# ubuntuslave/vo_single_camera_sos

Measured on AMD Instinct MI355X. Metric: frame-pairs/sec (detect+match+triangulate+RANSAC) on 640x480 omni, 2000 kpts, higher is better.
Workload: dtype u8/f32/f64

## Files before the change

vo_single_camera_sos_amd/csrc/ransac.hip:

```cpp
#include <type_traits>
#include "common.h"
#include "ransac_core.h"
#include "epnp_core.h"
#include "gp3p_core.h"

namespace {

constexpr int kMaxCam = 8;
constexpr int kHypDoubles = 16;
constexpr int kThreads = 256;
constexpr int kScoreHypChunkMax = 128;

__device__ const double kEye9[9] = {1, 0, 0, 0, 1, 0, 0, 0, 1};
__device__ const double kZero3[3] = {0, 0, 0};

__device__ __forceinline__ uint64_t problem_seed(uint64_t seed, int b) { return seed + (uint64_t)b; }
__device__ __forceinline__ uint64_t problem_seed(const uint64_t* seeds, int b) { return seeds[b]; }

__global__ __launch_bounds__(kThreads) void ransac_prepare_kernel(const int32_t* __restrict__ cam,
                                                                  const int32_t* __restrict__ n_arr, int stride,
                                                                  int ncam, int32_t* __restrict__ perm,
                                                                  int32_t* __restrict__ cinfo) {
  SOSVO_LATENCY_BOUND_PRIO();
  __shared__ int cnt[kThreads][kMaxCam];
  __shared__ int cstart[kMaxCam + 1];
  const int tid = threadIdx.x, b = blockIdx.x;
  const int n = min(n_arr[b], stride);
  const int chunk = (n + kThreads - 1) / kThreads;
  const int begin = min(n, tid * chunk), end = min(n, begin + chunk);
  const int32_t* camb = cam ? cam + (size_t)b * stride : nullptr;
  int local[kMaxCam];
#pragma unroll
  for (int c = 0; c < kMaxCam; ++c) local[c] = 0;
  for (int i = begin; i < end; ++i) {
    int c = camb ? camb[i] : 0;
    c = max(0, min(ncam - 1, c));
#pragma unroll
    for (int k = 0; k < kMaxCam; ++k) local[k] += (k == c);
  }
#pragma unroll
  for (int c = 0; c < kMaxCam; ++c) cnt[tid][c] = local[c];
  __syncthreads();
  if (tid < kMaxCam) {
    int running = 0;
    for (int t = 0; t < kThreads; ++t) {
      const int v = cnt[t][tid];
      cnt[t][tid] = running;
      running += v;
    }
    cinfo[(size_t)b * (2 * kMaxCam + 1) + kMaxCam + 1 + tid] = running;
    cstart[tid + 1] = running;
  }
  __syncthreads();
  if (tid == 0) {
    cstart[0] = 0;
    for (int c = 0; c < kMaxCam; ++c) cstart[c + 1] += cstart[c];
    for (int c = 0; c <= kMaxCam; ++c) cinfo[(size_t)b * (2 * kMaxCam + 1) + c] = cstart[c];
  }
  __syncthreads();
  int pos[kMaxCam];
#pragma unroll
  for (int c = 0; c < kMaxCam; ++c) pos[c] = cstart[c] + cnt[tid][c];
  for (int i = begin; i < end; ++i) {
    int c = camb ? camb[i] : 0;
    c = max(0, min(ncam - 1, c));
    int dst = 0;
#pragma unroll
    for (int k = 0; k < kMaxCam; ++k) {
      if (k == c) {
        dst = pos[k];
        pos[k] += 1;
      }
    }
    perm[(size_t)b * stride + dst] = i;
  }
}

__device__ __forceinline__ bool hyp_block(int nprob, int chunks, int* b, int* chunk) {
  const int xcd = (int)(blockIdx.x & 7), slot = (int)(blockIdx.x >> 3);
  *b = (slot / chunks) * 8 + xcd;
  *chunk = slot - (slot / chunks) * chunks;
  return *b < nprob;
}
static inline unsigned hyp_grid(int nprob, int chunks) { return (unsigned)(8 * cdiv(nprob, 8) * chunks); }

__device__ __forceinline__ void hyp_store_wave(double* __restrict__ hyp_b, int it0, int H, bool ok, const double* R,
                                               const double* t) {
  __shared__ double sh[64 * 17];
  const int lane = threadIdx.x;
  double* row = sh + lane * 17;
#pragma unroll
  for (int k = 0; k < 9; ++k) row[k] = ok ? R[k] : (k == 0 ? __longlong_as_double(0x7FF8000000000000LL) : 0.0);
#pragma unroll
  for (int k = 0; k < 3; ++k) row[9 + k] = ok ? t[k] : 0.0;
  row[12] = ok ? -(((R[0] * t[0]) + (R[3] * t[1])) + (R[6] * t[2])) : 0.0;
  row[13] = ok ? -(((R[1] * t[0]) + (R[4] * t[1])) + (R[7] * t[2])) : 0.0;
  row[14] = ok ? -(((R[2] * t[0]) + (R[5] * t[1])) + (R[8] * t[2])) : 0.0;
  row[15] = 0.0;
  __syncthreads();
#pragma unroll
  for (int j = 0; j < 16; ++j) {
    const int idx = j * 64 + lane, rec = idx >> 4, e = idx & 15;
    if (it0 + rec < H) hyp_b[(size_t)(it0 + rec) * kHypDoubles + e] = sh[rec * 17 + e];
  }
}

template <class SeedT>
__global__ __launch_bounds__(64) void ransac_hyp_kernel(const double* __restrict__ f, const double* __restrict__ p,
                                                        const int32_t* __restrict__ cam,
                                                        const double* __restrict__ cam_off,
                                                        const double* __restrict__ cam_rot,
                                                        const int32_t* __restrict__ n_arr, int nprob, int stride, int H,
                                                        SeedT seed, const int32_t* __restrict__ perm,
                                                        const int32_t* __restrict__ cinfo, double* __restrict__ hyp,
                                                        int32_t* __restrict__ counts) {
  SOSVO_LATENCY_BOUND_PRIO();
  int b, chunk;
  if (!hyp_block(nprob, (H + 63) >> 6, &b, &chunk)) return;
  const int it = chunk * 64 + threadIdx.x;
  const int n = min(n_arr[b], stride);
  const size_t base = (size_t)b * stride;
  const int32_t* ci = cinfo + (size_t)b * (2 * kMaxCam + 1);
  const double* off = cam ? cam_off : kZero3;
  const double* rot = cam ? cam_rot : kEye9;
  double R[9], t[3];
  int ok = 0;
  if (it < H)
    ok = sv_hypothesis(f + 3 * base, p + 3 * base, cam ? cam + base : nullptr, off, rot, n, perm + base, ci, ci + kMaxCam + 1,
                       problem_seed(seed, b), (uint64_t)it, R, t);
  hyp_store_wave(hyp + (size_t)b * H * kHypDoubles, chunk * 64, H, ok != 0, R, t);
  if (it < H) counts[(size_t)b * H + it] = ok ? 0 : -1;
}

template <class SeedT>
__global__ __launch_bounds__(64) void ransac_hyp_twopt_kernel(const double* __restrict__ f, const double* __restrict__ p,
                                                              const int32_t* __restrict__ n_arr, int nprob, int stride,
                                                              int H, SeedT seed, double* __restrict__ hyp,
                                                              int32_t* __restrict__ counts) {
  int b, chunk;
  if (!hyp_block(nprob, (H + 63) >> 6, &b, &chunk)) return;
// ... 70 lines not shown
      for (int k = 0; k < 48; ++k) out[k] = vv[k];
    }
  }
  counts[(size_t)b * H + it] = ok ? 0 : -1;
}

template <class SeedT>
__global__ __launch_bounds__(64) void ransac_epnp_pose_kernel(const double* __restrict__ f, const double* __restrict__ p,
                                                              const int32_t* __restrict__ n_arr, int nprob, int stride,
                                                              int H, SeedT seed, const double* __restrict__ vvbuf,
                                                              double* __restrict__ hyp, int32_t* __restrict__ counts) {
  SOSVO_LATENCY_BOUND_PRIO();
  int b, chunk;
  if (!hyp_block(nprob, (H + 63) >> 6, &b, &chunk)) return;
  const int it = chunk * 64 + threadIdx.x;
  const int n = min(n_arr[b], stride);
  double R[9], t[3];
  int ok = it < H && counts[(size_t)b * H + it] == 0;
  if (ok) {
    double p6[18], uv[2 * SV_EPNP_MAXN], cw[12], alphas[4 * SV_EPNP_MAXN], vv[48];
    ok = epnp_sample_front(f, p, n, (size_t)b * stride, problem_seed(seed, b), it, p6, uv, cw, alphas);
    const double* in = vvbuf + ((size_t)b * H + it) * kEpnpVecDoubles;
#pragma unroll
    for (int k = 0; k < 48; ++k) vv[k] = in[k];
    if (ok) ok = sv_epnp_back(p6, 6, uv, cw, alphas, vv, R, t);
  }
  hyp_store_wave(hyp + (size_t)b * H * kHypDoubles, chunk * 64, H, ok != 0, R, t);
  if (it < H) counts[(size_t)b * H + it] = ok ? 0 : -1;
}

template <bool IDENT>
__device__ __forceinline__ bool inlier_exact(const double* __restrict__ h, const double fx, const double fy,
                                             const double fz, const double px, const double py, const double pz,
                                             const double ox, const double oy, const double oz, const double* Rc,
                                             const double thr) {
  const double vx = (((h[0] * px) + (h[3] * py)) + (h[6] * pz)) + h[12];
  const double vy = (((h[1] * px) + (h[4] * py)) + (h[7] * pz)) + h[13];
  const double vz = (((h[2] * px) + (h[5] * py)) + (h[8] * pz)) + h[14];
  const double wx = vx - ox, wy = vy - oy, wz = vz - oz;
  double ux = wx, uy = wy, uz = wz;
  if (!IDENT) {
    ux = ((Rc[0] * wx) + (Rc[3] * wy)) + (Rc[6] * wz);
    uy = ((Rc[1] * wx) + (Rc[4] * wy)) + (Rc[7] * wz);
    uz = ((Rc[2] * wx) + (Rc[5] * wy)) + (Rc[8] * wz);
  }
  const double nrm = sqrt(((ux * ux) + (uy * uy)) + (uz * uz));
  const double gx = ux / nrm, gy = uy / nrm, gz = uz / nrm;
  return (1.0 - (((fx * gx) + (fy * gy)) + (fz * gz))) < thr;
}

constexpr double kTier1K = 1048576.0;
constexpr double kTier1Eps = 5.9604644775390625e-08;
constexpr double kTier1QBand = 3.47 / kTier1K + 20.0 * kTier1Eps;
constexpr double kTier1Max = 1e9;
constexpr double kTier1E2 = (3.47 * kTier1K + 6.0) * 78.03 * kTier1Eps * kTier1Eps * (1.0 + 1e-4);

__device__ __forceinline__ float score_tier1_lane(double fx, double fy, double fz, double px, double py, double pz, double ox,
                                                  double oy, double oz) {
  const double p1 = fabs(px) + fabs(py) + fabs(pz);
  const double om = fmax(fabs(ox), fmax(fabs(oy), fabs(oz)));
  const double fn = fx * fx + fy * fy + fz * fz;
  const double l = (p1 * p1 + om * om) * (1.0 + 1e-6);
  return (fabs(fn - 1.0) <= 1e-6 && p1 <= kTier1Max && om <= kTier1Max) ? (float)l : __builtin_inff();
}

__device__ __forceinline__ void score_tier1_hyp(const double* __restrict__ h, float* __restrict__ hs) {
  double rho = 0.0;
#pragma unroll
  for (int k = 0; k < 9; ++k) {
    hs[k] = (float)h[k];
    rho = fmax(rho, fabs(h[k]));
  }
  const double im = fmax(fabs(h[9]), fmax(fabs(h[10]), fabs(h[11])));
  hs[9] = (float)h[9], hs[10] = (float)h[10], hs[11] = (float)h[11];
  const double chk = (((((((h[0] + h[1]) + h[2]) + h[3]) + h[4]) + h[5]) + h[6]) + h[7]) + h[8] + h[9] + h[10] + h[11];
  const double ea = kTier1E2 * fmax(rho * rho, 1.0) * (1.0 + 1e-6);
  const double eb = kTier1E2 * (im * im) * (1.0 + 1e-6) + 1e-24;
  const bool fin = chk == chk && rho <= kTier1Max && im <= kTier1Max;
  hs[12] = fin ? (float)ea : __builtin_nanf("");
  hs[13] = fin ? (float)eb : __builtin_nanf("");
  hs[14] = 0.0f, hs[15] = 0.0f;
}

template <bool IDENT, int PPT, bool T1>
__global__ __launch_bounds__(kThreads) __attribute__((amdgpu_waves_per_eu(T1 ? 4 : 1))) void ransac_score_kernel(
    const double* __restrict__ f, const double* __restrict__ p, const int32_t* __restrict__ cam,
    const double* __restrict__ cam_off, const double* __restrict__ cam_rot, const int32_t* __restrict__ n_arr,
    int stride, int H, int hchunk, int hspan, double thr, int fast_ok, const double* __restrict__ hyp,
    int32_t* __restrict__ counts, int set_lo, int set_hi, int hsplit, const int32_t* __restrict__ alive_idx,
    const int32_t* __restrict__ n_alive) {
  static_assert(!T1 || (IDENT && PPT <= 4), "tier 1 is written for the identity-rotation form");
  SOSVO_LATENCY_BOUND_PRIO();
  constexpr bool KEEP = !T1;
  __shared__ int lcnt[kScoreHypChunkMax];
  __shared__ double shyp[kScoreHypChunkMax][12];
  __shared__ unsigned long long sok[(kScoreHypChunkMax + 63) / 64];
  __shared__ int sidx[kScoreHypChunkMax];
  __shared__ int srec[kScoreHypChunkMax];
  __shared__ float shyp32[T1 ? kScoreHypChunkMax : 1][16];
  const int tid = threadIdx.x, b = blockIdx.z;
  const int n = min(n_arr[b], stride);
  const int Hb = alive_idx ? n_alive[b] : H;
  const int xspan = alive_idx ? (int)((blockIdx.x + blockIdx.z) % gridDim.x) : (int)blockIdx.x;
  if (xspan * hspan >= Hb) return;
  const int sbeg = set_lo, send = min((n + 63) >> 6, set_hi);
  const int nsets = send - sbeg;
  const int bcap = hsplit ? PPT : (kThreads / 64) * PPT;
  const int nb = (nsets + bcap - 1) / bcap;
  if ((int)blockIdx.y >= nb) return;
  const int spb = (nsets + nb - 1) / nb;
  const int set0 = hsplit ? sbeg + ((int)blockIdx.y * nsets) / nb : sbeg + (int)blockIdx.y * spb;
  const int set1 = hsplit ? sbeg + (((int)blockIdx.y + 1) * nsets) / nb : min(set0 + spb, send);
  const int p0 = set0 * 64;

  double fx[KEEP ? PPT : 1], fy[KEEP ? PPT : 1], fz[KEEP ? PPT : 1];
  double px[KEEP ? PPT : 1], py[KEEP ? PPT : 1], pz[KEEP ? PPT : 1];
  double ox[KEEP ? PPT : 1], oy[KEEP ? PPT : 1], oz[KEEP ? PPT : 1];
  float fxs[T1 ? PPT : 1], fys[T1 ? PPT : 1], fzs[T1 ? PPT : 1], pxs[T1 ? PPT : 1], pys[T1 ? PPT : 1], pzs[T1 ? PPT : 1];
  float oxs[T1 ? PPT : 1], oys[T1 ? PPT : 1], ozs[T1 ? PPT : 1], lerr[T1 ? PPT : 1];
  int rowi[PPT];
  double Rc[IDENT ? 1 : 9];
  const int wave = __builtin_amdgcn_readfirstlane(tid >> 6), lane = tid & 63;
  const int wslot = (wave + blockIdx.x + blockIdx.y + blockIdx.z) & (kThreads / 64 - 1);
  const int jstep = hsplit ? kThreads / 64 : 1, jbeg = hsplit ? wslot : 0;
  const size_t base = (size_t)b * stride;
  unsigned long long vmask[PPT];
  int nlive_v = 0;
#pragma unroll
  for (int r = 0; r < PPT; ++r) {
    const int set = set0 + (hsplit ? r : r * (kThreads / 64) + wslot);
    const int i0 = set * 64;
    const int i = i0 + lane;
    nlive_v += set < set1 ? 1 : 0;
    const bool valid = i < n;
    vmask[r] = __ballot(valid);
    rowi[r] = valid ? i : p0;
    const size_t row = base + rowi[r];
    const double lfx = f[3 * row + 0], lfy = f[3 * row + 1], lfz = f[3 * row + 2];
    const double lpx = p[3 * row + 0], lpy = p[3 * row + 1], lpz = p[3 * row + 2];
    const int c = cam ? cam[row] : 0;
    const double* o = cam ? cam_off + 3 * c : kZero3;
    const double lox = o[0], loy = o[1], loz = o[2];
    if (KEEP) {
      fx[r] = lfx, fy[r] = lfy, fz[r] = lfz;
      px[r] = lpx, py[r] = lpy, pz[r] = lpz;
      ox[r] = lox, oy[r] = loy, oz[r] = loz;
    }
    if (!IDENT) {
      const double* rc = cam ? cam_rot + 9 * c : kEye9;
#pragma unroll
      for (int k = 0; k < 9; ++k) Rc[k] = rc[k];
    }
    if (T1) {
      fxs[r] = (float)lfx, fys[r] = (float)lfy, fzs[r] = (float)lfz;
      pxs[r] = (float)lpx, pys[r] = (float)lpy, pzs[r] = (float)lpz;
      oxs[r] = (float)lox, oys[r] = (float)loy, ozs[r] = (float)loz;
      lerr[r] = score_tier1_lane(lfx, lfy, lfz, lpx, lpy, lpz, lox, loy, loz);
    }
  }
  const int nlive = __builtin_amdgcn_readfirstlane(nlive_v);
  const double c1 = 1.0 - thr;
  const double c2 = c1 * c1;
  const double c2hi = c2 * (1.0 + 1e-9), c2lo = c2 * (1.0 - 1e-9);
  const float c2hs = (float)((c2 + kTier1QBand) * (1.0 + 1e-6)), c2ls = (float)((c2 - kTier1QBand) * (1.0 - 1e-6));
  const int hend = min(Hb, (xspan + 1) * hspan);
  for (int h0 = xspan * hspan; h0 < hend; h0 += hchunk) {
  const int h1 = min(hend, h0 + hchunk);
  for (int k = tid; k < kScoreHypChunkMax; k += kThreads) lcnt[k] = 0;
  const int nh = h1 - h0;
  const double* hb = hyp + (size_t)b * H * kHypDoubles;
  static_assert(kScoreHypChunkMax == 128, "two words of solved-hypothesis flags");
  if (wave < 2) {
    const int hh = wave * 64 + lane;
    const int rec = hh < nh ? (alive_idx ? alive_idx[(size_t)b * H + h0 + hh] : h0 + hh) : 0;
    const double r00 = hh < nh ? hb[(size_t)rec * kHypDoubles] : 0.0;
    const unsigned long long okb = __ballot(hh < nh && r00 == r00);
    if (lane == 0) sok[wave] = okb;
    srec[hh] = rec;
  }
  __syncthreads();
  const unsigned long long ok0 = sok[0], ok1 = sok[1];
  const int nok = __builtin_amdgcn_readfirstlane(__popcll(ok0) + __popcll(ok1));
  for (int k = tid; k < nh * 12; k += kThreads) {
    const int hh = k / 12, e = k - hh * 12;
    const unsigned long long w = hh < 64 ? ok0 : ok1;
    if ((w >> (hh & 63)) & 1ULL) {
      const int pos = __popcll(w & ((1ULL << (hh & 63)) - 1ULL)) + (hh < 64 ? 0 : __popcll(ok0));
      const int rec = srec[hh];
      shyp[pos][e] = hb[(size_t)rec * kHypDoubles + (e < 9 ? e : e + 3)];
      if (e == 0) sidx[pos] = rec;
    }
  }
  __syncthreads();
  if (T1) {
    for (int pos = tid; pos < nok; pos += kThreads) score_tier1_hyp(shyp[pos], shyp32[pos]);
    __syncthreads();
  }

  auto tier2 = [&](auto nl, const int j, const unsigned long long* und1) -> int {
    constexpr int NL = decltype(nl)::value;
    int total = 0;
    const double* hp = shyp[j];
    const double r0 = hp[0], r1 = hp[1], r2 = hp[2], r3 = hp[3], r4 = hp[4], r5 = hp[5], r6 = hp[6], r7 = hp[7], r8 = hp[8];
    const double ix = hp[9], iy = hp[10], iz = hp[11];
#pragma unroll
    for (int r = 0; r < NL && r < PPT; ++r) {
      if (!und1[r]) continue;
      double Fx, Fy, Fz, Px, Py, Pz, Ox, Oy, Oz;
      if (KEEP) {
        Fx = fx[r], Fy = fy[r], Fz = fz[r], Px = px[r], Py = py[r], Pz = pz[r];
        Ox = ox[r], Oy = oy[r], Oz = oz[r];
      } else {
        const size_t row = base + rowi[r];
        Fx = f[3 * row + 0], Fy = f[3 * row + 1], Fz = f[3 * row + 2];
        Px = p[3 * row + 0], Py = p[3 * row + 1], Pz = p[3 * row + 2];
        const double* o = cam ? cam_off + 3 * cam[row] : kZero3;
// ... 21 lines not shown
      }
      if (und) {
        const double vx = (((r0 * Px) + (r3 * Py)) + (r6 * Pz)) + ix;
        const double vy = (((r1 * Px) + (r4 * Py)) + (r7 * Pz)) + iy;
        const double vz = (((r2 * Px) + (r5 * Py)) + (r8 * Pz)) + iz;
        const double wx = vx - Ox, wy = vy - Oy, wz = vz - Oz;
        double ux = wx, uy = wy, uz = wz;
        if (!IDENT) {
          ux = ((Rc[0] * wx) + (Rc[IDENT ? 0 : 3] * wy)) + (Rc[IDENT ? 0 : 6] * wz);
          uy = ((Rc[IDENT ? 0 : 1] * wx) + (Rc[IDENT ? 0 : 4] * wy)) + (Rc[IDENT ? 0 : 7] * wz);
          uz = ((Rc[IDENT ? 0 : 2] * wx) + (Rc[IDENT ? 0 : 5] * wy)) + (Rc[IDENT ? 0 : 8] * wz);
        }
        const double q = ((ux * ux) + (uy * uy)) + (uz * uz);
        const double nrm = sqrt(q);
        const double gx = ux / nrm, gy = uy / nrm, gz = uz / nrm;
        total += __popcll(__ballot((1.0 - (((Fx * gx) + (Fy * gy)) + (Fz * gz))) < thr) & und);
      }
    }
    return total;
  };

  auto tier1 = [&](auto nl, const int j, unsigned long long* und1, unsigned long long& any1) -> int {
    constexpr int NL = decltype(nl)::value;
    int total = 0;
    const float* hs = shyp32[T1 ? j : 0];
    const float q0 = hs[0], q1 = hs[1], q2 = hs[2], q3 = hs[3], q4 = hs[4], q5 = hs[5], q6 = hs[6], q7 = hs[7], q8 = hs[8];
    const float jx = hs[9], jy = hs[10], jz = hs[11], ea = hs[12], eb = hs[13];
#pragma unroll
    for (int r = 0; r < NL && r < PPT; ++r) {
      const float ux = fmaf(q0, pxs[T1 ? r : 0], fmaf(q3, pys[T1 ? r : 0], fmaf(q6, pzs[T1 ? r : 0], jx - oxs[T1 ? r : 0])));
      const float uy = fmaf(q1, pxs[T1 ? r : 0], fmaf(q4, pys[T1 ? r : 0], fmaf(q7, pzs[T1 ? r : 0], jy - oys[T1 ? r : 0])));
      const float uz = fmaf(q2, pxs[T1 ? r : 0], fmaf(q5, pys[T1 ? r : 0], fmaf(q8, pzs[T1 ? r : 0], jz - ozs[T1 ? r : 0])));
      const float sv = fmaf(fxs[T1 ? r : 0], ux, fmaf(fys[T1 ? r : 0], uy, fzs[T1 ? r : 0] * uz));
      const float qv = fmaf(ux, ux, fmaf(uy, uy, uz * uz));
      const float lhs = sv * fabsf(sv);
      const float e2 = fmaf(ea, lerr[T1 ? r : 0], eb);
      const unsigned long long hi = __ballot(lhs > fmaf(c2hs, qv, e2));
      const unsigned long long lo = __ballot(lhs < fmaf(c2ls, qv, -e2));
      total += __popcll(hi & vmask[r]);
      und1[r] = ~hi & ~lo & vmask[r];
      any1 |= und1[r];
    }
    return total;
  };

  auto hyp_loop = [&](auto nl) {
    constexpr int NL = decltype(nl)::value;
    int cntv = 0, k = 0;
    for (int j = jbeg; j < nok; j += jstep, ++k) {
      unsigned long long und[PPT], any = 0ULL;
      int tot = 0;
      if (T1) {
        tot = tier1(nl, j, und, any);
      } else {
#pragma unroll
        for (int r = 0; r < NL && r < PPT; ++r) {
          und[r] = vmask[r];
          any |= vmask[r];
        }
      }
      if (any) tot += tier2(nl, j, und);
      if (lane == (k & 63)) cntv += tot;
      if ((k & 63) == 63) {
        if (cntv) atomicAdd(&lcnt[jbeg + ((k & ~63) + lane) * jstep], cntv);
        cntv = 0;
      }
    }
    if (cntv) atomicAdd(&lcnt[jbeg + (((k - 1) & ~63) + lane) * jstep], cntv);
  };
  if (nlive >= 4) hyp_loop(std::integral_constant<int, 4>{});
  else if (nlive == 3) hyp_loop(std::integral_constant<int, 3>{});
  else if (nlive == 2) hyp_loop(std::integral_constant<int, 2>{});
  else if (nlive == 1) hyp_loop(std::integral_constant<int, 1>{});
  __syncthreads();
  for (int k = tid; k < nok; k += kThreads) {
    const int v = lcnt[k];
    if (v) atomicAdd(&counts[(size_t)b * H + sidx[k]], v);
  }
  }
}

__global__ __launch_bounds__(kThreads) void ransac_prune_kernel(
    const double* __restrict__ f, const double* __restrict__ p, const int32_t* __restrict__ cam,
    const double* __restrict__ cam_off, const int32_t* __restrict__ n_arr, int stride, int H, int probe_sets, double thr,
    const double* __restrict__ hyp, const int32_t* __restrict__ counts, int32_t* __restrict__ alive_idx,
    int32_t* __restrict__ n_alive) {
  SOSVO_LATENCY_BOUND_PRIO();
  __shared__ long long red[kThreads / 64];
  __shared__ int redc[kThreads / 64];
  __shared__ int wave_off[kThreads / 64 + 1];
  const int tid = threadIdx.x, b = blockIdx.x, lane = tid & 63, wid = tid >> 6;
  const int n = min(n_arr[b], stride);
  const int32_t* cb = counts + (size_t)b * H;
  int32_t* ab = alive_idx + (size_t)b * H;
  long long best_key = -1;
  for (int it = tid; it < H; it += kThreads) {
    const int c = cb[it];
    const long long key = ((long long)c << 32) | (long long)(0x7FFFFFFF - it);
    if (c >= 0 && key > best_key) best_key = key;
  }
  for (int o = 32; o > 0; o >>= 1) {
    const long long other = __shfl_down(best_key, o);
    best_key = other > best_key ? other : best_key;
  }
  if (lane == 0) red[wid] = best_key;
  __syncthreads();
  best_key = red[0];
  for (int w = 1; w < kThreads / 64; ++w) best_key = red[w] > best_key ? red[w] : best_key;
  if (best_key < 0) {
    if (tid == 0) n_alive[b] = 0;
    return;
  }
  const int hstar = 0x7FFFFFFF - (int)(best_key & 0xFFFFFFFFLL);
  const double* hp = hyp + ((size_t)b * H + hstar) * kHypDoubles;
  const size_t base = (size_t)b * stride;
  int cnt = 0;
  for (int i = tid; i < n; i += kThreads) {
    const size_t row = base + i;
    const double* o = cam ? cam_off + 3 * cam[row] : kZero3;
    cnt += inlier_exact<true>(hp, f[3 * row], f[3 * row + 1], f[3 * row + 2], p[3 * row], p[3 * row + 1], p[3 * row + 2], o[0],
                              o[1], o[2], kEye9, thr) ? 1 : 0;
  }
  for (int o = 32; o > 0; o >>= 1) cnt += __shfl_down(cnt, o);
  if (lane == 0) redc[wid] = cnt;
  __syncthreads();
  const int L = ((redc[0] + redc[1]) + redc[2]) + redc[3];
  const int rest = n - min(n, probe_sets * 64);
  int running = 0;
  for (int it0 = 0; it0 < H; it0 += kThreads) {
    const int it = it0 + tid;
    const int c = it < H ? cb[it] : -1;
    const bool keep = c >= 0 && c + rest >= L;
    const unsigned long long bal = __ballot(keep);
    __syncthreads();
    if (lane == 0) wave_off[wid + 1] = __popcll(bal);
    __syncthreads();
    int off = running;
    for (int w = 0; w < wid; ++w) off += wave_off[w + 1];
    if (keep) ab[off + __popcll(bal & ((1ULL << lane) - 1ULL))] = it;
    running += ((wave_off[1] + wave_off[2]) + wave_off[3]) + wave_off[4];
  }
  if (tid == 0) n_alive[b] = running;
}

template <bool IDENT>
__global__ __launch_bounds__(kThreads) void ransac_select_kernel(
    const double* __restrict__ f, const double* __restrict__ p, const int32_t* __restrict__ cam,
    const double* __restrict__ cam_off, const double* __restrict__ cam_rot, const int32_t* __restrict__ n_arr,
    int stride, int H, double thr, int adaptive, const double* __restrict__ hyp, const int32_t* __restrict__ counts,
    double* __restrict__ T_out, uint8_t* __restrict__ mask, int32_t* __restrict__ inl_idx,
    int32_t* __restrict__ n_inl, int32_t* __restrict__ info) {
  SOSVO_LATENCY_BOUND_PRIO();
  __shared__ long long red[kThreads / 64];
  __shared__ int redv[kThreads / 64];
  __shared__ int s_best_it, s_used, s_nvalid;
  __shared__ int wave_off[kThreads / 64 + 1];
  __shared__ int s_running;
  const int tid = threadIdx.x, b = blockIdx.x, lane = tid & 63, wid = tid >> 6;
  const int n = min(n_arr[b], stride);
  const int32_t* cb = counts + (size_t)b * H;

  long long best_key = -1;
  int nvalid = 0;
  for (int it = tid; it < H; it += kThreads) {
    const int c = cb[it];
    if (c >= 0) {
      nvalid++;
      const long long key = ((long long)c << 32) | (long long)(0x7FFFFFFF - it);
      best_key = key > best_key ? key : best_key;
    }
  }
  for (int o = 32; o > 0; o >>= 1) {
    const long long other = __shfl_down(best_key, o);
    best_key = other > best_key ? other : best_key;
    nvalid += __shfl_down(nvalid, o);
  }
  if (lane == 0) {
    red[wid] = best_key;
    redv[wid] = nvalid;
  }
  __syncthreads();
  if (tid == 0) {
    long long k = red[0];
    int nv = redv[0];
    for (int w = 1; w < kThreads / 64; ++w) {
      k = red[w] > k ? red[w] : k;
      nv += redv[w];
    }
    s_nvalid = nv;
    if (!(adaptive & 1)) {
      s_best_it = k < 0 ? -1 : (0x7FFFFFFF - (int)(k & 0xFFFFFFFFLL));
      s_used = H;
    } else {
      int best_count = -1, best_it = -1, iterations = 0, used = 0;
      double base = 1.0;
      for (int it = 0; it < H; ++it) {
        if (iterations > 0 && !sv_ransac_continue(base, iterations)) break;
        used = it + 1;
        const int c = cb[it];
        if (c < 0) continue;
        if (c > best_count) {
          best_count = c;
          best_it = it;
          base = (adaptive & 2) ? sv_adaptive_base6(c, n) : ((adaptive & 4) ? sv_adaptive_base2(c, n) : sv_adaptive_base(c, n));
        }
        iterations++;
      }
      s_best_it = best_it;
      s_used = used;
    }
    s_running = 0;
  }
  __syncthreads();
  const int best_it = s_best_it;
  const size_t base = (size_t)b * stride;
  if (best_it < 0) {
    for (int i = tid; i < n; i += kThreads) mask[base + i] = 0;
    if (tid < 12) T_out[(size_t)b * 12 + tid] = (tid == 0 || tid == 5 || tid == 10) ? 1.0 : 0.0;
    if (tid == 0) {
      n_inl[b] = 0;
      info[4 * b + 0] = -1;
      info[4 * b + 1] = s_used;
      info[4 * b + 2] = 1;
      info[4 * b + 3] = s_nvalid;
    }
// ... 165 lines not shown
      for (int q = tid; q < cnt; q += kThreads) {
        const int i = idx ? idx[base + q] : q;
        const size_t row = base + i;
        const int cc = cam ? cam[row] : 0;
        const double* o = cam ? cam_off + 3 * cc : kZero3;
        const double* rc = cam ? cam_rot + 9 * cc : kEye9;
        const double r = sv_residual(xn, f + 3 * row, p + 3 * row, o, rc);
        cn += r * r;
      }
      cn = block_sum(cn, scratch, tid);
      if (cn < cost) {
        converged = ((cost - cn) <= SV_LM_FTOL * cost);
        __syncthreads();
        if (tid == 0) {
#pragma unroll
          for (int u = 0; u < 6; ++u) sx[u] = xn[u];
        }
        cost = cn;
        lambda *= 0.1;
        if (lambda < 1e-15) lambda = 1e-15;
        accepted = 1;
        __syncthreads();
        break;
      }
      lambda *= 10.0;
      __syncthreads();
    }
    it_done = it + 1;
    if (!accepted || converged) break;
  }
  __syncthreads();
  if (tid == 0) {
    double R[9], t[3];
    sv_cayley2rot(sx + 3, R);
    t[0] = sx[0];
    t[1] = sx[1];
    t[2] = sx[2];
    sv_Rt_to_T(R, t, T);
    if (cost_out) cost_out[b] = cost;
    if (iters_out) iters_out[b] = it_done;
  }
}

}

template <class SeedT>
static int32_t ransac_abs_pose_impl(sosvo_ctx* ctx, const char* fn, const double* f, const double* p, const int32_t* cam,
                                    const double* cam_off, const double* cam_rot, int32_t ncam, int32_t flags,
                                    const int32_t* n, int32_t nprob, int32_t stride, double thr, int32_t max_iter,
                                    int32_t adaptive, SeedT seed, double* T_out,
                                    uint8_t* inlier_mask, int32_t* inlier_idx, int32_t* n_inliers, int32_t* info,
                                    int32_t* hyp_counts) {
#define SOSVO_LAUNCH_HYP(ctx, kernel, ...)              \
  do {                                                  \
    SOSVO_PROFILE(ctx, #kernel);                        \
    hipLaunchKernelGGL((kernel<SeedT>), __VA_ARGS__);   \
  } while (0)
#define SOSVO_REQUIRE_FN(ctx, cond, msg)                               \
  do {                                                                 \
    if (!(cond)) return sosvo_fail((ctx), SOSVO_ERR_ARG, fn, msg);     \
  } while (0)
  SOSVO_REQUIRE_FN(ctx, f && p && n && T_out && inlier_mask && inlier_idx && n_inliers && info, "null pointer");
  SOSVO_REQUIRE_FN(ctx, cam == nullptr || (cam_off && cam_rot), "cam given without cam_off / cam_rot");
  SOSVO_REQUIRE_FN(ctx, ncam >= 1 && ncam <= kMaxCam, "ncam out of range (1..8)");
  SOSVO_REQUIRE_FN(ctx, nprob >= 0 && nprob <= 65535, "nprob out of range");
  SOSVO_REQUIRE_FN(ctx, stride > 0 && stride <= (1 << 20), "stride out of range");
  SOSVO_REQUIRE_FN(ctx, max_iter > 0 && max_iter <= (1 << 20), "max_iter out of range");
  SOSVO_REQUIRE_FN(ctx, thr > 0.0, "threshold must be positive");
  if (nprob == 0) return SOSVO_OK;
  const int H = max_iter;
  size_t off = 0;
  auto carve = [&](size_t bytes) {
    size_t o = off;
    off += (bytes + 255) & ~(size_t)255;
    return o;
  };
  const size_t o_perm = carve(sizeof(int32_t) * (size_t)nprob * stride);
  const size_t o_cinfo = carve(sizeof(int32_t) * (size_t)nprob * (2 * kMaxCam + 1));
  const size_t o_hyp = carve(sizeof(double) * (size_t)nprob * H * kHypDoubles);
  const size_t o_counts = carve(sizeof(int32_t) * (size_t)nprob * H);
  const bool epnp_vec = (flags & SOSVO_FLAG_EPNP) != 0;
  const size_t o_vv = carve(epnp_vec ? sizeof(double) * (size_t)nprob * H * kEpnpVecDoubles : 0);
  const size_t o_alive = carve(sizeof(int32_t) * (size_t)nprob * (H + 1));
  int32_t rc = sosvo_ws_reserve(ctx, off);
  if (rc != SOSVO_OK) return rc;
  char* ws = (char*)ctx->ws;
  int32_t* perm = (int32_t*)(ws + o_perm);
  int32_t* cinfo = (int32_t*)(ws + o_cinfo);
  double* hyp = (double*)(ws + o_hyp);
  int32_t* counts = hyp_counts ? hyp_counts : (int32_t*)(ws + o_counts);

  SOSVO_LAUNCH(ctx,ransac_prepare_kernel, dim3(nprob), dim3(kThreads), 0, ctx->stream, cam, n, stride,
                     cam ? ncam : 1, perm, cinfo);
  SOSVO_LAUNCH_CHECK(ctx);
  const int epnp = (flags & SOSVO_FLAG_EPNP) != 0;
  SOSVO_REQUIRE_FN(ctx, !epnp || cam == nullptr, "SOSVO_FLAG_EPNP is for central problems (cam == NULL)");
  const int twopt = (flags & SOSVO_FLAG_TWOPT) != 0 && !epnp && !(flags & SOSVO_FLAG_GP3P);
  SOSVO_REQUIRE_FN(ctx, !twopt || cam == nullptr, "SOSVO_FLAG_TWOPT is for central problems (cam == NULL)");
  if (epnp) adaptive = (adaptive ? 1 : 0) | 2;
  if (twopt) adaptive = (adaptive ? 1 : 0) | 4;
  if (epnp) {
    double* vvbuf = (double*)(ws + o_vv);
    SOSVO_LAUNCH_HYP(ctx, ransac_epnp_eigen_kernel, dim3(hyp_grid(nprob, cdiv(H, 64))), dim3(64), 0, ctx->stream, f, p, n, nprob, stride, H,
                 seed, vvbuf, counts);
    SOSVO_LAUNCH_HYP(ctx, ransac_epnp_pose_kernel, dim3(hyp_grid(nprob, cdiv(H, 64))), dim3(64), 0, ctx->stream, f, p, n, nprob, stride, H,
                 seed, vvbuf, hyp, counts);
  } else if (twopt) {
    SOSVO_LAUNCH_HYP(ctx, ransac_hyp_twopt_kernel, dim3(hyp_grid(nprob, cdiv(H, 64))), dim3(64), 0, ctx->stream, f, p, n, nprob, stride, H, seed,
                 hyp, counts);
  } else if (flags & SOSVO_FLAG_GP3P) {
    SOSVO_LAUNCH_HYP(ctx, ransac_hyp_gp3p_kernel, dim3(hyp_grid(nprob, cdiv(H, 64))), dim3(64), 0, ctx->stream, f, p, cam, cam_off, cam_rot,
                 n, nprob, stride, H, seed, hyp, counts);
  } else
    SOSVO_LAUNCH_HYP(ctx, ransac_hyp_kernel, dim3(hyp_grid(nprob, cdiv(H, 64))), dim3(64), 0, ctx->stream, f, p, cam, cam_off, cam_rot, n,
                 nprob, stride, H, seed, perm, cinfo, hyp, counts);
  SOSVO_LAUNCH_CHECK(ctx);

  const bool ident = (flags & SOSVO_FLAG_CAM_ROT_IDENTITY) != 0 || cam == nullptr;
  const int fast_ok = thr < 0.5 ? 1 : 0;
  const int ppt = ident ? 4 : 1;
  const int gx = cdiv(stride, kThreads * ppt);
  const bool t1 = ident && fast_ok && !ctx->hint_score_fp64_only;
  const int wg_target = t1 ? 4096 : 8192;
  int hchunks = cdiv(wg_target, nprob);
  if (hchunks < 1) hchunks = 1;
  int hspan = cdiv(H, hchunks);
  if (hspan < 32) hspan = H < 32 ? H : 32;
  hchunks = cdiv(H, hspan);
  const int hchunk = cdiv(hspan, cdiv(hspan, kScoreHypChunkMax));
  dim3 grid(hchunks, gx, nprob);
  constexpr int kProbeSets = 4, kPruneMinSets = 8, kPruneMinProblems = 64;
  const bool prune = t1 && adaptive == 0 && hyp_counts == nullptr && !epnp && !twopt && stride >= 64 * kPruneMinSets &&
                     nprob >= kPruneMinProblems;
#define SOSVO_SCORE_ARGS grid, dim3(kThreads), 0, ctx->stream, f, p, cam, cam_off, cam_rot, n, stride, H, hchunk, hspan, thr, fast_ok, hyp, counts, 0, INT_MAX, 0, (const int32_t*)nullptr, (const int32_t*)nullptr
  if (prune) {
    int32_t* alive_idx = (int32_t*)(ws + o_alive);
    int32_t* n_alive = alive_idx + (size_t)nprob * H;
    auto pass = [&](int set_lo, int set_hi, int hs, const int32_t* list, const int32_t* nlist) {
      const int hck = cdiv(hs, cdiv(hs, kScoreHypChunkMax));
      const int sets = min(set_hi, cdiv(stride, 64)) - set_lo;
      SOSVO_LAUNCH(ctx,(ransac_score_kernel<true, 4, true>), dim3(cdiv(H, hs), cdiv(sets, 4), nprob), dim3(kThreads), 0,
                   ctx->stream, f, p, cam, cam_off, cam_rot, n, stride, H, hck, hs, thr, fast_ok, hyp, counts, set_lo, set_hi, 1,
                   list, nlist);
    };
    pass(0, kProbeSets, min(H, 4 * hspan), nullptr, nullptr);
    SOSVO_LAUNCH(ctx,ransac_prune_kernel, dim3(nprob), dim3(kThreads), 0, ctx->stream, f, p, cam, cam_off, n, stride, H,
                 kProbeSets, thr, hyp, counts, alive_idx, n_alive);
    pass(kProbeSets, INT_MAX, min(H, max(kScoreHypChunkMax, 2 * hspan)), alive_idx, n_alive);
  } else if (t1)
    SOSVO_LAUNCH(ctx,(ransac_score_kernel<true, 4, true>), SOSVO_SCORE_ARGS);
  else if (ident)
    SOSVO_LAUNCH(ctx,(ransac_score_kernel<true, 4, false>), SOSVO_SCORE_ARGS);
  else
    SOSVO_LAUNCH(ctx,(ransac_score_kernel<false, 1, false>), SOSVO_SCORE_ARGS);
#undef SOSVO_SCORE_ARGS
  SOSVO_LAUNCH_CHECK(ctx);
  if (ident)
    SOSVO_LAUNCH(ctx,(ransac_select_kernel<true>), dim3(nprob), dim3(kThreads), 0, ctx->stream, f, p, cam,
                       cam_off, cam_rot, n, stride, H, thr, adaptive, hyp, counts, T_out, inlier_mask, inlier_idx,
                       n_inliers, info);
  else
    SOSVO_LAUNCH(ctx,(ransac_select_kernel<false>), dim3(nprob), dim3(kThreads), 0, ctx->stream, f, p, cam,
                       cam_off, cam_rot, n, stride, H, thr, adaptive, hyp, counts, T_out, inlier_mask, inlier_idx,
                       n_inliers, info);
  SOSVO_LAUNCH_CHECK(ctx);
  return SOSVO_OK;
}
#undef SOSVO_REQUIRE_FN
#undef SOSVO_LAUNCH_HYP

extern "C" {

int32_t sosvo_ransac_abs_pose(sosvo_ctx* ctx, const double* f, const double* p, const int32_t* cam,
                              const double* cam_off, const double* cam_rot, int32_t ncam, int32_t flags,
                              const int32_t* n, int32_t nprob, int32_t stride, double thr, int32_t max_iter,
                              int32_t adaptive, uint64_t seed, double* T_out, uint8_t* inlier_mask,
                              int32_t* inlier_idx, int32_t* n_inliers, int32_t* info, int32_t* hyp_counts) {
  SOSVO_ENTER(ctx);
  return ransac_abs_pose_impl(ctx, __func__, f, p, cam, cam_off, cam_rot, ncam, flags, n, nprob, stride, thr, max_iter, adaptive,
                              seed, T_out, inlier_mask, inlier_idx, n_inliers, info, hyp_counts);
}

int32_t sosvo_ransac_abs_pose_seeds(sosvo_ctx* ctx, const double* f, const double* p, const int32_t* cam,
                                    const double* cam_off, const double* cam_rot, int32_t ncam, int32_t flags,
                                    const int32_t* n, int32_t nprob, int32_t stride, double thr, int32_t max_iter,
                                    int32_t adaptive, const uint64_t* seeds, double* T_out, uint8_t* inlier_mask,
                                    int32_t* inlier_idx, int32_t* n_inliers, int32_t* info, int32_t* hyp_counts) {
  SOSVO_ENTER(ctx);
  SOSVO_REQUIRE(ctx, seeds, "null seed array");
  return ransac_abs_pose_impl(ctx, __func__, f, p, cam, cam_off, cam_rot, ncam, flags, n, nprob, stride, thr, max_iter, adaptive,
                              seeds, T_out, inlier_mask, inlier_idx, n_inliers, info, hyp_counts);
}

int32_t sosvo_refine_abs_pose(sosvo_ctx* ctx, const double* f, const double* p, const int32_t* cam,
                              const double* cam_off, const double* cam_rot, int32_t ncam, const int32_t* n,
                              int32_t nprob, int32_t stride, const int32_t* idx, const int32_t* m,
                              int32_t max_lm_iter, double* T_io, double* cost_out, int32_t* iters_out) {
  SOSVO_ENTER(ctx);
  SOSVO_REQUIRE(ctx, f && p && n && T_io, "null pointer");
  SOSVO_REQUIRE(ctx, cam == nullptr || (cam_off && cam_rot), "cam given without cam_off / cam_rot");
  SOSVO_REQUIRE(ctx, (idx == nullptr) == (m == nullptr), "idx and m go together");
  SOSVO_REQUIRE(ctx, ncam >= 1 && ncam <= kMaxCam, "ncam out of range (1..8)");
  SOSVO_REQUIRE(ctx, nprob >= 0 && nprob <= 65535, "nprob out of range");
  SOSVO_REQUIRE(ctx, stride > 0 && stride <= (1 << 20), "stride out of range");
  SOSVO_REQUIRE(ctx, max_lm_iter > 0 && max_lm_iter <= 10000, "max_lm_iter out of range");
  if (nprob == 0) return SOSVO_OK;
  SOSVO_LAUNCH(ctx,refine_kernel, dim3(nprob), dim3(kThreads), 0, ctx->stream, f, p, cam, cam_off, cam_rot, n,
                     stride, idx, m, max_lm_iter, T_io, cost_out, iters_out);
  SOSVO_LAUNCH_CHECK(ctx);
  return SOSVO_OK;
}

}
```

Before: 70690.

## Add multi-stage RANSAC hypothesis pruning with camera-split-aware set ordering

Extends the single probe-then-prune scoring scheme to several stages (plan 4, 14 sets). A prune kernel runs after each stage and narrows the list of surviving hypotheses incrementally, and it only recomputes the best hypothesis's exact inlier count when the leader has changed. The prepare kernel also records where the camera index first changes in each problem. Scoring then visits point sets in an interleaved order from both ends of that split, so the probe sets cover both camera groups and give tighter bounds earlier. This adds extra kernel launches and workspace buffers, and the gain depends on how many hypotheses can be discarded early.

```diff
diff --git a/vo_single_camera_sos_amd/csrc/ransac.hip b/vo_single_camera_sos_amd/csrc/ransac.hip
--- a/vo_single_camera_sos_amd/csrc/ransac.hip
+++ b/vo_single_camera_sos_amd/csrc/ransac.hip
@@ -20,27 +20,34 @@
 __global__ __launch_bounds__(kThreads) void ransac_prepare_kernel(const int32_t* __restrict__ cam,
                                                                   const int32_t* __restrict__ n_arr, int stride,
                                                                   int ncam, int32_t* __restrict__ perm,
-                                                                  int32_t* __restrict__ cinfo) {
+                                                                  int32_t* __restrict__ cinfo,
+                                                                  int32_t* __restrict__ split_out) {
   SOSVO_LATENCY_BOUND_PRIO();
   __shared__ int cnt[kThreads][kMaxCam];
   __shared__ int cstart[kMaxCam + 1];
+  __shared__ int s_split;
   const int tid = threadIdx.x, b = blockIdx.x;
   const int n = min(n_arr[b], stride);
+  if (tid == 0) s_split = n;
   const int chunk = (n + kThreads - 1) / kThreads;
   const int begin = min(n, tid * chunk), end = min(n, begin + chunk);
   const int32_t* camb = cam ? cam + (size_t)b * stride : nullptr;
   int local[kMaxCam];
 #pragma unroll
   for (int c = 0; c < kMaxCam; ++c) local[c] = 0;
+  const int c0 = camb && n > 0 ? max(0, min(ncam - 1, camb[0])) : 0;
+  int other = n;
   for (int i = begin; i < end; ++i) {
     int c = camb ? camb[i] : 0;
     c = max(0, min(ncam - 1, c));
 #pragma unroll
     for (int k = 0; k < kMaxCam; ++k) local[k] += (k == c);
+    if (c != c0) other = min(other, i);
   }
 #pragma unroll
   for (int c = 0; c < kMaxCam; ++c) cnt[tid][c] = local[c];
   __syncthreads();
+  if (other < n) atomicMin(&s_split, other);
   if (tid < kMaxCam) {
     int running = 0;
     for (int t = 0; t < kThreads; ++t) {
@@ -56,6 +63,7 @@
     cstart[0] = 0;
     for (int c = 0; c < kMaxCam; ++c) cstart[c + 1] += cstart[c];
     for (int c = 0; c <= kMaxCam; ++c) cinfo[(size_t)b * (2 * kMaxCam + 1) + c] = cstart[c];
+    split_out[b] = s_split;
   }
   __syncthreads();
   int pos[kMaxCam];
@@ -292,13 +300,20 @@
   hs[14] = 0.0f, hs[15] = 0.0f;
 }
 
+__device__ __forceinline__ int score_set_at(int E, int n, int split, int k) {
+  if (split <= 0 || split >= n) return E - 1 - k;
+  const int tb = split >> 6, nbot = E - 1 - tb, ntop = tb + 1, m = min(nbot, ntop);
+  if (k < 2 * m) return (k & 1) ? tb - (k >> 1) : E - 1 - (k >> 1);
+  return nbot > ntop ? E - 1 - (k - m) : tb - (k - m);
+}
+
 template <bool IDENT, int PPT, bool T1>
 __global__ __launch_bounds__(kThreads) __attribute__((amdgpu_waves_per_eu(T1 ? 4 : 1))) void ransac_score_kernel(
     const double* __restrict__ f, const double* __restrict__ p, const int32_t* __restrict__ cam,
     const double* __restrict__ cam_off, const double* __restrict__ cam_rot, const int32_t* __restrict__ n_arr,
     int stride, int H, int hchunk, int hspan, double thr, int fast_ok, const double* __restrict__ hyp,
     int32_t* __restrict__ counts, int set_lo, int set_hi, int hsplit, const int32_t* __restrict__ alive_idx,
-    const int32_t* __restrict__ n_alive) {
+    const int32_t* __restrict__ n_alive, const int32_t* __restrict__ split_arr) {
   static_assert(!T1 || (IDENT && PPT <= 4), "tier 1 is written for the identity-rotation form");
   SOSVO_LATENCY_BOUND_PRIO();
   constexpr bool KEEP = !T1;
@@ -313,7 +328,9 @@
   const int Hb = alive_idx ? n_alive[b] : H;
   const int xspan = alive_idx ? (int)((blockIdx.x + blockIdx.z) % gridDim.x) : (int)blockIdx.x;
   if (xspan * hspan >= Hb) return;
-  const int sbeg = set_lo, send = min((n + 63) >> 6, set_hi);
+  const int nset_all = (n + 63) >> 6, split = split_arr ? split_arr[b] : 0;
+  auto set_at = [&](int k) { return split_arr ? score_set_at(nset_all, n, split, k) : k; };
+  const int sbeg = set_lo, send = min(nset_all, set_hi);
   const int nsets = send - sbeg;
   const int bcap = hsplit ? PPT : (kThreads / 64) * PPT;
   const int nb = (nsets + bcap - 1) / bcap;
@@ -321,7 +338,7 @@
   const int spb = (nsets + nb - 1) / nb;
   const int set0 = hsplit ? sbeg + ((int)blockIdx.y * nsets) / nb : sbeg + (int)blockIdx.y * spb;
   const int set1 = hsplit ? sbeg + (((int)blockIdx.y + 1) * nsets) / nb : min(set0 + spb, send);
-  const int p0 = set0 * 64;
+  const int p0 = set_at(set0) * 64;
 
   double fx[KEEP ? PPT : 1], fy[KEEP ? PPT : 1], fz[KEEP ? PPT : 1];
   double px[KEEP ? PPT : 1], py[KEEP ? PPT : 1], pz[KEEP ? PPT : 1];
@@ -338,10 +355,10 @@
   int nlive_v = 0;
 #pragma unroll
   for (int r = 0; r < PPT; ++r) {
-    const int set = set0 + (hsplit ? r : r * (kThreads / 64) + wslot);
-    const int i0 = set * 64;
+    const int pos = set0 + (hsplit ? r : r * (kThreads / 64) + wslot);
+    const int i0 = (pos < set1 ? set_at(pos) : nset_all) * 64;
     const int i = i0 + lane;
-    nlive_v += set < set1 ? 1 : 0;
+    nlive_v += pos < set1 ? 1 : 0;
     const bool valid = i < n;
     vmask[r] = __ballot(valid);
     rowi[r] = valid ? i : p0;
@@ -529,9 +546,10 @@
 
 __global__ __launch_bounds__(kThreads) void ransac_prune_kernel(
     const double* __restrict__ f, const double* __restrict__ p, const int32_t* __restrict__ cam,
-    const double* __restrict__ cam_off, const int32_t* __restrict__ n_arr, int stride, int H, int probe_sets, double thr,
-    const double* __restrict__ hyp, const int32_t* __restrict__ counts, int32_t* __restrict__ alive_idx,
-    int32_t* __restrict__ n_alive) {
+    const double* __restrict__ cam_off, const int32_t* __restrict__ n_arr, int stride, int H, int k_done, double thr,
+    const double* __restrict__ hyp, const int32_t* __restrict__ counts, const int32_t* __restrict__ in_idx,
+    const int32_t* __restrict__ n_in, int32_t* __restrict__ alive_idx, int32_t* __restrict__ n_alive,
+    int32_t* __restrict__ state) {
   SOSVO_LATENCY_BOUND_PRIO();
   __shared__ long long red[kThreads / 64];
   __shared__ int redc[kThreads / 64];
@@ -539,9 +557,12 @@
   const int tid = threadIdx.x, b = blockIdx.x, lane = tid & 63, wid = tid >> 6;
   const int n = min(n_arr[b], stride);
   const int32_t* cb = counts + (size_t)b * H;
+  const int32_t* ib = in_idx ? in_idx + (size_t)b * H : nullptr;
   int32_t* ab = alive_idx + (size_t)b * H;
+  const int Hin = in_idx ? n_in[b] : H;
   long long best_key = -1;
-  for (int it = tid; it < H; it += kThreads) {
+  for (int j = tid; j < Hin; j += kThreads) {
+    const int it = ib ? ib[j] : j;
     const int c = cb[it];
     const long long key = ((long long)c << 32) | (long long)(0x7FFFFFFF - it);
     if (c >= 0 && key > best_key) best_key = key;
@@ -559,24 +580,29 @@
     return;
   }
   const int hstar = 0x7FFFFFFF - (int)(best_key & 0xFFFFFFFFLL);
-  const double* hp = hyp + ((size_t)b * H + hstar) * kHypDoubles;
-  const size_t base = (size_t)b * stride;
-  int cnt = 0;
-  for (int i = tid; i < n; i += kThreads) {
-    const size_t row = base + i;
-    const double* o = cam ? cam_off + 3 * cam[row] : kZero3;
-    cnt += inlier_exact<true>(hp, f[3 * row], f[3 * row + 1], f[3 * row + 2], p[3 * row], p[3 * row + 1], p[3 * row + 2], o[0],
-                              o[1], o[2], kEye9, thr) ? 1 : 0;
-  }
-  for (int o = 32; o > 0; o >>= 1) cnt += __shfl_down(cnt, o);
-  if (lane == 0) redc[wid] = cnt;
-  __syncthreads();
-  const int L = ((redc[0] + redc[1]) + redc[2]) + redc[3];
-  const int rest = n - min(n, probe_sets * 64);
+  const int L_prev = in_idx ? state[2 * b] : 0, h_prev = in_idx ? state[2 * b + 1] : -1;
+  int L = L_prev;
+  if (hstar != h_prev) {
+    const double* hp = hyp + ((size_t)b * H + hstar) * kHypDoubles;
+    const size_t base = (size_t)b * stride;
+    int cnt = 0;
+    for (int i = tid; i < n; i += kThreads) {
+      const size_t row = base + i;
+      const double* o = cam ? cam_off + 3 * cam[row] : kZero3;
+      cnt += inlier_exact<true>(hp, f[3 * row], f[3 * row + 1], f[3 * row + 2], p[3 * row], p[3 * row + 1], p[3 * row + 2],
+                                o[0], o[1], o[2], kEye9, thr) ? 1 : 0;
+    }
+    for (int o = 32; o > 0; o >>= 1) cnt += __shfl_down(cnt, o);
+    if (lane == 0) redc[wid] = cnt;
+    __syncthreads();
+    L = max(L_prev, ((redc[0] + redc[1]) + redc[2]) + redc[3]);
+  }
+  const int rest = 64 * max(0, ((n + 63) >> 6) - k_done);
   int running = 0;
-  for (int it0 = 0; it0 < H; it0 += kThreads) {
-    const int it = it0 + tid;
-    const int c = it < H ? cb[it] : -1;
+  for (int j0 = 0; j0 < Hin; j0 += kThreads) {
+    const int j = j0 + tid;
+    const int it = j < Hin ? (ib ? ib[j] : j) : 0;
+    const int c = j < Hin ? cb[it] : -1;
     const bool keep = c >= 0 && c + rest >= L;
     const unsigned long long bal = __ballot(keep);
     __syncthreads();
@@ -587,7 +613,11 @@
     if (keep) ab[off + __popcll(bal & ((1ULL << lane) - 1ULL))] = it;
     running += ((wave_off[1] + wave_off[2]) + wave_off[3]) + wave_off[4];
   }
-  if (tid == 0) n_alive[b] = running;
+  if (tid == 0) {
+    n_alive[b] = running;
+    state[2 * b] = L;
+    state[2 * b + 1] = hstar;
+  }
 }
 
 template <bool IDENT>
@@ -919,6 +949,9 @@
   const bool epnp_vec = (flags & SOSVO_FLAG_EPNP) != 0;
   const size_t o_vv = carve(epnp_vec ? sizeof(double) * (size_t)nprob * H * kEpnpVecDoubles : 0);
   const size_t o_alive = carve(sizeof(int32_t) * (size_t)nprob * (H + 1));
+  const size_t o_alive2 = carve(sizeof(int32_t) * (size_t)nprob * (H + 1));
+  const size_t o_stage = carve(sizeof(int32_t) * (size_t)nprob * 2);
+  const size_t o_split = carve(sizeof(int32_t) * (size_t)nprob);
   int32_t rc = sosvo_ws_reserve(ctx, off);
   if (rc != SOSVO_OK) return rc;
   char* ws = (char*)ctx->ws;
@@ -926,9 +959,10 @@
   int32_t* cinfo = (int32_t*)(ws + o_cinfo);
   double* hyp = (double*)(ws + o_hyp);
   int32_t* counts = hyp_counts ? hyp_counts : (int32_t*)(ws + o_counts);
+  int32_t* split = (int32_t*)(ws + o_split);
 
   SOSVO_LAUNCH(ctx,ransac_prepare_kernel, dim3(nprob), dim3(kThreads), 0, ctx->stream, cam, n, stride,
-                     cam ? ncam : 1, perm, cinfo);
+                     cam ? ncam : 1, perm, cinfo, split);
   SOSVO_LAUNCH_CHECK(ctx);
   const int epnp = (flags & SOSVO_FLAG_EPNP) != 0;
   SOSVO_REQUIRE_FN(ctx, !epnp || cam == nullptr, "SOSVO_FLAG_EPNP is for central problems (cam == NULL)");
@@ -966,24 +1000,44 @@
   hchunks = cdiv(H, hspan);
   const int hchunk = cdiv(hspan, cdiv(hspan, kScoreHypChunkMax));
   dim3 grid(hchunks, gx, nprob);
-  constexpr int kProbeSets = 4, kPruneMinSets = 8, kPruneMinProblems = 64;
+  constexpr int kProbeSets = 4, kPruneMinSets = 8, kStageMinSets = 16, kPruneMinProblems = 64;
+#ifndef SOSVO_STAGE_PLAN
+#define SOSVO_STAGE_PLAN 4, 14
+#endif
+  static const int kStagePlan[] = {SOSVO_STAGE_PLAN};
   const bool prune = t1 && adaptive == 0 && hyp_counts == nullptr && !epnp && !twopt && stride >= 64 * kPruneMinSets &&
                      nprob >= kPruneMinProblems;
-#define SOSVO_SCORE_ARGS grid, dim3(kThreads), 0, ctx->stream, f, p, cam, cam_off, cam_rot, n, stride, H, hchunk, hspan, thr, fast_ok, hyp, counts, 0, INT_MAX, 0, (const int32_t*)nullptr, (const int32_t*)nullptr
+#define SOSVO_SCORE_ARGS grid, dim3(kThreads), 0, ctx->stream, f, p, cam, cam_off, cam_rot, n, stride, H, hchunk, hspan, thr, fast_ok, hyp, counts, 0, INT_MAX, 0, (const int32_t*)nullptr, (const int32_t*)nullptr, (const int32_t*)nullptr
   if (prune) {
-    int32_t* alive_idx = (int32_t*)(ws + o_alive);
-    int32_t* n_alive = alive_idx + (size_t)nprob * H;
-    auto pass = [&](int set_lo, int set_hi, int hs, const int32_t* list, const int32_t* nlist) {
+    const int capsets = cdiv(stride, 64);
+    const bool staged = stride >= 64 * kStageMinSets;
+    int nstage = 1;
+    if (staged)
+      for (nstage = 0; nstage < (int)(sizeof(kStagePlan) / sizeof(kStagePlan[0])) && kStagePlan[nstage] < capsets;) ++nstage;
+    int32_t* alive_idx[2] = {(int32_t*)(ws + o_alive), (int32_t*)(ws + o_alive2)};
+    int32_t* stage_state = (int32_t*)(ws + o_stage);
+    auto pass = [&](int k_lo, int k_hi, const int32_t* list) {
+      const int sets = min(k_hi, capsets) - k_lo;
+      int hs = min(H, (sets <= 4 ? 4 : 2) * hspan);
+      if (list) hs = min(H, max(kScoreHypChunkMax, hs));
       const int hck = cdiv(hs, cdiv(hs, kScoreHypChunkMax));
-      const int sets = min(set_hi, cdiv(stride, 64)) - set_lo;
       SOSVO_LAUNCH(ctx,(ransac_score_kernel<true, 4, true>), dim3(cdiv(H, hs), cdiv(sets, 4), nprob), dim3(kThreads), 0,
-                   ctx->stream, f, p, cam, cam_off, cam_rot, n, stride, H, hck, hs, thr, fast_ok, hyp, counts, set_lo, set_hi, 1,
-                   list, nlist);
+                   ctx->stream, f, p, cam, cam_off, cam_rot, n, stride, H, hck, hs, thr, fast_ok, hyp, counts, k_lo, k_hi, 1,
+                   list, list ? list + (size_t)nprob * H : nullptr, split);
     };
-    pass(0, kProbeSets, min(H, 4 * hspan), nullptr, nullptr);
-    SOSVO_LAUNCH(ctx,ransac_prune_kernel, dim3(nprob), dim3(kThreads), 0, ctx->stream, f, p, cam, cam_off, n, stride, H,
-                 kProbeSets, thr, hyp, counts, alive_idx, n_alive);
-    pass(kProbeSets, INT_MAX, min(H, max(kScoreHypChunkMax, 2 * hspan)), alive_idx, n_alive);
+    int k_lo = 0;
+    const int32_t* list = nullptr;
+    for (int s = 0; s < nstage; ++s) {
+      const int k_hi = staged ? kStagePlan[s] : kProbeSets;
+      pass(k_lo, k_hi, list);
+      int32_t* out = alive_idx[s & 1];
+      SOSVO_LAUNCH(ctx,ransac_prune_kernel, dim3(nprob), dim3(kThreads), 0, ctx->stream, f, p, cam, cam_off, n, stride, H,
+                   k_hi, thr, hyp, counts, list, list ? list + (size_t)nprob * H : nullptr, out, out + (size_t)nprob * H,
+                   stage_state);
+      list = out;
+      k_lo = k_hi;
+    }
+    pass(k_lo, INT_MAX, list);
   } else if (t1)
     SOSVO_LAUNCH(ctx,(ransac_score_kernel<true, 4, true>), SOSVO_SCORE_ARGS);
   else if (ident)
```

After: 72400 (median of 6 runs). 1.02x the previous value.
